# acoustic-warfare/beamforming-lk

Hardware: AMD Instinct MI355X
Metric: heatmap frames/sec (higher is better)
Workload: dtype f32

## Files before the change

### beamforming-lk_amd/csrc/awpu_handle.h

```cpp
#pragma once

#include "awpu_hip.h"
#include "awpu_hip_spectral.h"
#include "awpu_hip_track.h"

#include <hip/hip_runtime.h>

#include <algorithm>
#include <string>
#include <utility>
#include <vector>

#include "das_kernels.h"

namespace awpu::host {

void note_error(const std::string &text);

struct CtxScope {
    awpu_hip *saved;
    explicit CtxScope(awpu_hip *h);
    ~CtxScope();
};
#define AWPU_CTX(h) awpu::host::CtxScope ctx_scope_(h)
// ... 177 lines not shown
}

struct awpu_hip {
    template <class T>
    using Dev = awpu::host::DeviceBuffer<T>;
    template <class T>
    using Pinned = awpu::host::PinnedBuffer<T>;
    using Event = awpu::host::Event;
    using Stream = awpu::host::Stream;

    awpu_hip_cfg cfg{};
    Stream stream;
    Event ev_begin, ev_end;
    bool timing = true;

    std::vector<int32_t> off;
    std::vector<float> frac;
    std::vector<int32_t> index;
    std::vector<float> gain;
    bool have_table = false, have_mics = false, prepared = false;

    Dev<awpu::LutEntry> d_lut;
    struct FastLut {
        awpu::FastPlan plan;
        Dev<awpu::FastEntry> d;
        size_t entries = 0;
    };
    std::vector<FastLut> fast_luts;
    Dev<awpu::FastEntry> d_exact_pair_lut;
    size_t exact_pair_lut_entries = 0, fir_plane_lut_entries = 0;
    awpu::FastPlan exact_plan{};
    awpu::host::QuadTable quad_tables[awpu::host::kQuadLayouts];
    Dev<unsigned> d_nd_queue;
    Dev<int2> d_nd_items;
    Dev<unsigned> d_nd_starts;
    size_t nd_start_entries = 0;
    long long nd_items_key = -1;
    int n_cus = 0;
    bool exact_nd_ok = false;
    bool exact_ndh_ok = false, exact_ndhs_ok = false, fast_ndp_ok = false;
    bool identity_mics = false;
    bool exact_pairs_ok = false;
    float *sums_out = nullptr;
    Dev<uint32_t> d_fir_plane_lut;
    awpu::FastPlan fir_plane_plan{};
    bool fir_planes_ok = false;
    std::vector<float> fir;
    bool quadh_fits = false;
    bool quadhs_fits = false;
    bool quad_ok = false;
    double quad_cost = 0.0;
    double quad_differ = 3.0;
    Dev<int32_t> d_index;
    Dev<float> d_gain;
    Dev<float> d_calib;
    Dev<awpu::LutEntry> d_beam_lut;
    Dev<float> d_beam_out;
    std::vector<float> antenna;
    Dev<float> d_xyz;
    std::vector<int32_t> track_index;
    Dev<int32_t> d_track_index;
    Dev<unsigned char> d_track;
    Dev<float> d_fir;
    Dev<float> d_ring;
    Dev<uint8_t> d_display;
    Dev<awpu::ResizeTap> d_taps;
    int taps_key[4] = {0, 0, 0, 0};
// ... 63 lines not shown
};

namespace awpu::host {

enum class ExactShape : int {
    kVerify = 0,
    kDefault = 1,
    kPair = 2,
    kQuad = 3,
    kNd1 = 4,
    kNd2 = 5,
    kNdp = 6,
};
inline bool forces_exact_nd(ExactShape e) { return e == ExactShape::kNd1 || e == ExactShape::kNd2 || e == ExactShape::kNdp; }

struct EnvKnobs {
    int fpi = 0, ppw = 0, nw = 0;
    int pairs = -1;
    int debug = 0;
    int fpw = 0;
    int quads = -1;
    int pair_group = 0;
    int quad_variant = 0;
    int stationary = -1;
    int fir_planes = 1;
    int fir_share = 1;
    int wgs = 0;
    int live_graph = 1;
    int halves = -1;
    ExactShape exact_pairs = ExactShape::kDefault;
    int pair_cols = -1;
    int group_copy = 0;
    int listen_stream = 1;
    EnvKnobs();
};
const EnvKnobs &env();

struct BandSet {
    int n = 0;
    int taps[AWPU_SPECTRAL_MAX_BANDS] = {0, 0, 0, 0};
    const float *coef[AWPU_SPECTRAL_MAX_BANDS] = {nullptr, nullptr, nullptr, nullptr};
    int max_taps() const { return std::max(std::max(taps[0], taps[1]), std::max(taps[2], taps[3])); }
    int planes() const { return std::max(n, 1); }
};
inline BandSet own_band(const awpu_hip *h) {
    BandSet set;
    if (!h->band.empty()) set.n = 1, set.taps[0] = h->band_taps(), set.coef[0] = h->band.data();
    return set;
}

enum FrameLayout { kFull = 0, kCompact = 1, kRing = 2 };

int prepare(awpu_hip *h);
void free_tables(awpu_hip *h);
int launch(awpu_hip *h, const float *d_frames, int batch, float *d_power, hipStream_t s, int layout = kFull);
bool takes_packed_pairs(awpu_hip *h, int batch, awpu::FastPlan *plan);
int packed_shape(awpu_hip *h, int batch, awpu::FastPlan *plan);
size_t packed_floats_of(const awpu_hip *h, const awpu::FastPlan &plan, int batch);
int pack_for_sweep(awpu_hip *h, const awpu::FastPlan &plan, const float *d_frames, int batch, float *d_packed, hipStream_t s);
int sweep_packed(awpu_hip *h, const awpu::FastPlan &plan, const float *d_packed, size_t packed_floats, int batch, float *d_power, hipStream_t s);

void retire_live_graphs(awpu_hip *h);
int enqueue_host_process(awpu_hip *h, const float *frames, int batch, const BandSet *bands = nullptr);
int enqueue_power_to_host(awpu_hip *h, int batch, float *power, size_t pitch);
int enqueue_ingest(awpu_hip *h, const void *datagrams, int32_t stride_bytes);
int check_ready(awpu_hip *h, int batch);
// ... 52 lines not shown
```

### beamforming-lk_amd/csrc/awpu_hip.cpp

```cpp
#include "awpu_handle.h"

#include <algorithm>
#include <chrono>
#include <cmath>
#include <cstdio>
#include <cstdlib>
#include <cstring>
#include <new>
#include <string>
#include <vector>

#include "awpu_hip_band.h"
#include "band_kernels.h"
#include "band_rule.h"
#include "spectral_kernels.h"
#include "spectral_rule.h"
#include "das_kernels.h"
#include "focus_rule.h"
#include "watch_kernels.h"

using namespace awpu::host;

namespace {

// ... 3 lines not shown
}

namespace awpu::host {

void note_error(const std::string &text) {
    g_last_error = text;
    if (g_ctx) g_ctx->last_error = text;
}

CtxScope::CtxScope(awpu_hip *h) : saved(g_ctx) { g_ctx = h; }
CtxScope::~CtxScope() { g_ctx = saved; }

int hip_fail(hipError_t e, const char *what) {
    note_error(std::string(what) + ": " + hipGetErrorString(e));
    return AWPU_ERR_HIP;
}

int invalid(const char *why) {
    note_error(why);
    return AWPU_ERR_INVALID;
}

int fail(int status, const char *why) {
    note_error(why);
    return status;
}

}

awpu::host::EnvKnobs::EnvKnobs() {
    if (const char *v = std::getenv("AWPU_GROUP_FORCE_COPY")) group_copy = std::atoi(v);
    if (const char *v = std::getenv("AWPU_LIVE_GRAPH")) live_graph = std::atoi(v);
    if (const char *v = std::getenv("AWPU_SHAPE")) {
        const std::string shape(v);
        if (shape == "pair" || shape == "pair_vertical" || shape == "pair_horizontal") {
            pairs = 1, quads = 0, stationary = 0;
            if (shape != "pair") pair_cols = shape == "pair_vertical";
        } else if (shape == "quad") quads = 1;
        else if (shape == "noquad") quads = 0;
        else if (shape == "stationary") pairs = 1, quads = 0, stationary = 1;
        else if (shape == "quadh") quads = 1, pairs = 0, halves = 1;
        else if (shape == "quadh_chunked") quads = 1, pairs = 0, halves = 1, stationary = 0;
        else if (shape == "single_db") pairs = 0, quads = 0, fpi = 1, ppw = 8, nw = 32;
        else if (shape == "single_small") pairs = 0, quads = 0, fpi = 1, ppw = 2, nw = 8;
        else if (shape == "fir8_planes") fir_planes = 2;
        else if (shape == "exact_verify") exact_pairs = ExactShape::kVerify;
        else if (shape == "exact_pair") exact_pairs = ExactShape::kPair;
        else if (shape == "exact_quad") exact_pairs = ExactShape::kQuad;
        else if (shape == "exact_nd1") exact_pairs = ExactShape::kNd1;
        else if (shape == "exact_nd2") exact_pairs = ExactShape::kNd2;
        else if (shape == "exact_ndp") exact_pairs = ExactShape::kNdp;
        else std::fprintf(stderr, "libawpu_hip: AWPU_SHAPE=%s is not a shape of this build; ignored\n", v);
    }
#ifdef AWPU_TUNING_BUILD
    if (const char *v = std::getenv("AWPU_LISTEN_STREAM")) listen_stream = std::atoi(v);
    if (const char *v = std::getenv("AWPU_FAST_QUADS")) quads = std::atoi(v);
    if (const char *v = std::getenv("AWPU_FAST_PAIRGROUP")) pair_group = std::atoi(v);
    if (const char *v = std::getenv("AWPU_QUAD_VARIANT")) quad_variant = std::atoi(v);
    if (const char *v = std::getenv("AWPU_FAST_HALVES")) halves = std::atoi(v);
    if (const char *v = std::getenv("AWPU_EXACT_PAIRS")) exact_pairs = (ExactShape) std::atoi(v);
    if (const char *v = std::getenv("AWPU_FAST_WGS")) wgs = std::atoi(v);
    if (const char *v = std::getenv("AWPU_FIR8_PLANES")) fir_planes = std::atoi(v);
    if (const char *v = std::getenv("AWPU_FIR8_SHARE")) fir_share = std::atoi(v);
    if (const char *v = std::getenv("AWPU_FAST_STATIONARY")) stationary = std::atoi(v);
    if (const char *v = std::getenv("AWPU_FAST_PAIRCOLS")) pair_cols = std::atoi(v);
    if (const char *v = std::getenv("AWPU_FAST_VARIANT"))
        if (std::sscanf(v, "%d,%d,%d", &fpi, &ppw, &nw) < 2) fpi = ppw = nw = 0;
// ... 1239 lines not shown
```

### beamforming-lk_amd/csrc/awpu_sweep.cpp

```cpp
#include "awpu_handle.h"

#include <algorithm>
#include <array>
#include <cstdio>
#include <cstdlib>
#include <cstring>
#include <map>
#include <vector>

#include "das_kernels.h"
#include "nd_tile_window.h"

using namespace awpu::host;

namespace {

int diag_begin(awpu_hip *h, size_t words, bool zero, hipStream_t s, unsigned long long **out) {
    if (const int rc = h->d_diag.ensure(words); rc != AWPU_OK) return rc;
    if (zero) AWPU_HIP_TRY(hipMemsetAsync(h->d_diag, 0, words * sizeof(unsigned long long), s));
    *out = h->d_diag;
    return AWPU_OK;
}

int diag_end(awpu_hip *h, int rc, size_t n_waves, int wg_waves, const char *tag, hipStream_t s) {
// ... 440 lines not shown
    }
    if (env_fpi == 1 || env_fpi == 2) *fpi = env_fpi;
    if (env_ppw == 2 || env_ppw == 4 || env_ppw == 8) *ppw = env_ppw;
    if (env_nw == 8 || env_nw == 32 || env_nw == 24) *nw = env_nw;
    if (*nw == 32) {
        *fpi = 1;
        if (*ppw < 4) *ppw = 4;
    }
    if (*nw == 24) {
        *fpi = 1;
        *ppw = 4;
    }
    if (*fpi == 2 && *ppw == 8) *ppw = 4;
    if (*fpi == 2 && batch < 2) *fpi = 1;
}

int finish_launch(awpu_hip *h, int batch, hipStream_t s, int kernel_id) {
    h->stats.kernel_variant = kernel_id;
    if (h->timing) AWPU_HIP_TRY(hipEventRecord(h->ev_end, s));
    h->stats.launches += 1;
    h->stats.frames += (uint64_t) batch;
    return AWPU_OK;
}

int cu_count(awpu_hip *h) {
    if (h->n_cus < 1 && (hipDeviceGetAttribute(&h->n_cus, hipDeviceAttributeMultiprocessorCount, h->cfg.device) != hipSuccess || h->n_cus < 1))
        h->n_cus = 256;
    return h->n_cus;
}

int arm_item_queues(awpu_hip *h, int items, unsigned **queue, int32_t *wgs, int32_t *tail) {
    if (const int rc = h->d_nd_queue.ensure(9); rc != AWPU_OK) return rc;
    *queue = h->d_nd_queue;
    *wgs = cu_count(h);
    const int per = (items + 7) / 8;
    *tail = per >= 32 ? (per + 7) / 8 : per;
    return AWPU_OK;
}

size_t pair_pack_floats(int frames, int rows, int wr, int floats) { return (size_t) ((frames + 1) / 2) * rows * wr * floats; }

template <class Args>
void fill_shared(Args &a, const awpu_hip *h, const awpu::FastPlan &plan, int batch, float *d_power) {
    a.power = d_power;
    a.usable = h->usable();
    a.usable_pad = plan.usable_pad;
    a.pixel_count = h->cfg.pixel_count;
    a.chunk = plan.chunk;
    a.batch = batch;
}

int launch_exact_pairs(awpu_hip *h, const float *d_frames, int batch, float *d_power, hipStream_t s, int hist_eff, int wstart_eff) {
    if (const int rc = build_exact_pair_lut(h); rc != AWPU_OK) return rc;
    const awpu::FastPlan &pp = h->exact_plan;
    if (const int prc = ensure_pack(h, pair_pack_floats(std::max(h->cfg.max_batch, batch), pp.usable_pad, pp.wr, 2)); prc != AWPU_OK) return prc;
    awpu::ExactPairArgs a{};
    fill_shared(a, h, pp, batch, d_power);
    a.packed = h->d_pack;
    a.lut = h->d_exact_pair_lut;
    a.sums = h->sums_out;
    a.wp = pp.wr;
    a.cols = h->pair_cols;
    a.tiles = awpu::pair_tiles(a.pixel_count, a.cols);
    a.n_pairs = (batch + 1) / 2;
    a.pair_group = awpu::xcd_pair_group((size_t) pp.usable_pad * pp.wr * 8, a.n_pairs);
    if (h->timing) AWPU_HIP_TRY(hipEventRecord(h->ev_begin, s));
    AWPU_HIP_TRY(awpu::launch_pack_pairs(d_frames, h->cfg.n_streams, hist_eff, wstart_eff, h->d_index, h->usable(), pp.usable_pad,
// ... 580 lines not shown
```

### beamforming-lk_amd/csrc/das_fast.hip

```cpp
#include "das_kernels.h"

#include <algorithm>
#include <atomic>

namespace awpu {

typedef float f2 __attribute__((ext_vector_type(2)));
typedef float f4 __attribute__((ext_vector_type(4)));
typedef float f4u __attribute__((ext_vector_type(4), aligned(4)));
typedef float f8 __attribute__((ext_vector_type(8)));

#define AWPU_AS4 __attribute__((address_space(4)))

typedef int i16 __attribute__((ext_vector_type(16)));

struct EntryGroup {
    i16 v;
    __device__ __forceinline__ float f(int k) const { return __int_as_float(v[4 * k + 0]); }
    __device__ __forceinline__ unsigned addr(int k) const { return (unsigned) v[4 * k + 1]; }
    __device__ __forceinline__ float g(int k) const { return __int_as_float(v[4 * k + 2]); }
};

template <int FPI>
struct Reads {
// ... 159 lines not shown
}

__device__ __forceinline__ float sum8(float v) {
    v += dpp_take<0xB1>(v);
    v += dpp_take<0x4E>(v);
    v += dpp_take<0x141>(v);
    return v;
}
__device__ __forceinline__ float sum16(float v) {
    v = sum8(v);
    return v + dpp_take<0x140>(v);
}
__device__ __forceinline__ float sum32(float v) {
    v = sum16(v);
    return v + dpp_take<0x142, 0xa>(v);
}
template <int LPP>
__device__ __forceinline__ float sum_lanes(float v) {
    static_assert(LPP == 8 || LPP == 16 || LPP == 32, "groups of 8, 16 or 32 lanes");
    return LPP == 8 ? sum8(v) : LPP == 16 ? sum16(v) : sum32(v);
}
template <int LPP>
__device__ __forceinline__ constexpr int sum_lane_of(int group) {
    return LPP == 32 ? 32 * group + 16 : LPP * group;
}
__device__ __forceinline__ float lane_value(float v, int lane_index) {
    return __builtin_bit_cast(float, __builtin_amdgcn_readlane(__builtin_bit_cast(int, v), lane_index));
}

constexpr int kDppWaveRol1 = 0x134;
constexpr int kDppWaveRor1 = 0x13C;
template <int CTRL>
__device__ __forceinline__ float wave_rotate1(float v) {
    const int bits = __builtin_bit_cast(int, v);
    return __builtin_bit_cast(float, __builtin_amdgcn_update_dpp(bits, bits, CTRL, 0xf, 0xf, false));
}

__device__ __forceinline__ float finish_pixel(f2 A, f2 Q, f2 C, f2 R, float tail, int lane) {
    const float q_rot = wave_rotate1<kDppWaveRol1>(Q.x);
    const float r_rot = wave_rotate1<kDppWaveRol1>(R.x);
    const float q_next = lane == 63 ? r_rot : q_rot;
    const float r_next = lane == 63 ? tail : r_rot;
    const float o0 = A.x + Q.y;
    const float o1 = A.y + q_next;
    const float o2 = C.x + R.y;
    const float o3 = C.y + r_next;
    const float o1_prev = wave_rotate1<kDppWaveRor1>(o1);
    const float o2_next = wave_rotate1<kDppWaveRol1>(o2);
    const float o0_rot = wave_rotate1<kDppWaveRol1>(o0);
    const float o3_rot = wave_rotate1<kDppWaveRor1>(o3);
    const float o0_next = lane == 63 ? o2_next : o0_rot;
    const float o3_prev = lane == 0 ? o1_prev : o3_rot;
    const float ma0 = o0 * 0.5f - 0.25f * (o1 + o1_prev);
    const float ma1 = o1 * 0.5f - 0.25f * (o0_next + o0);
    const float ma2 = o2 * 0.5f - 0.25f * (o3 + o3_prev);
    const float ma3 = o3 * 0.5f - 0.25f * (o2_next + o2);
    float sum = ma1 * ma1 + ma2 * ma2;
    if (lane != 0) sum += ma0 * ma0;
    if (lane != 63) sum += ma3 * ma3;
    return wave_sum(sum);
}

template <int NW, int PPW, int FPI, int WPS>
__global__ __launch_bounds__(NW * 64, WPS) void das_fast_kernel(FastArgs a) {
    static_assert(PPW <= 8, "the tail pass gives 8 lanes to each of at most 8 pixels");
    extern __shared__ __attribute__((aligned(16))) float lds[];
    constexpr int FS = kFastLdsBytes / FPI;
    const int lane = threadIdx.x & 63;
// ... 854 lines not shown
    }
}

__device__ __forceinline__ f2 next_and_difference(float cur, float next, float gm) {
#pragma clang fp contract(off)
    const float c = cur * gm, n = next * gm;
    return f2{n, c - n};
}

__global__ void pack_nd_kernel(const float *frames, int n_streams, int hist, int wstart, const int32_t *index, int usable,
                               const float *gain, int wq, int batch, float *packed, unsigned *queue) {
    const int pair = blockIdx.y, s = blockIdx.x, rows_out = gridDim.x;
    if (queue && pair == 0 && s == 0 && threadIdx.x < 9) queue[threadIdx.x] = 0u;
    f4 *dst = (f4 *) packed + ((size_t) pair * rows_out + s) * wq;
    if (s >= usable) {
        for (int t = threadIdx.x; t < wq; t += blockDim.x) dst[t] = f4{0.0f, 0.0f, 0.0f, 0.0f};
        return;
    }
    const int fa = min(2 * pair, batch - 1), fb = min(2 * pair + 1, batch - 1);
    const float *xa = frames + ((size_t) fa * n_streams + index[s]) * hist + wstart;
    const float *xb = frames + ((size_t) fb * n_streams + index[s]) * hist + wstart;
    const float gm = gain ? gain[s] : 1.0f;
    const int valid = min(wq, hist - wstart - 1);
    for (int t = threadIdx.x; t < wq; t += blockDim.x) {
        f4 v = f4{0.0f, 0.0f, 0.0f, 0.0f};
        if (t < valid) {
            const f2 ea = next_and_difference(xa[t], xa[t + 1], gm), eb = next_and_difference(xb[t], xb[t + 1], gm);
            v = f4{ea.x, eb.x, ea.y, eb.y};
        }
        dst[t] = v;
    }
}

__global__ void nd_items_kernel(int2 *items, int n_pairs, int tiles, int pair_group, int tiles_per_row, int nq) {
    const int item = blockIdx.x * blockDim.x + threadIdx.x;
    if (item >= n_pairs * tiles) return;
    const int full_items = (n_pairs / pair_group) * pair_group * tiles;
    const int ga = item < full_items ? pair_group : n_pairs % pair_group;
    const int rem = item < full_items ? item : item - full_items;
    const int grp = rem / (tiles * ga), in = rem - grp * tiles * ga;
    const int tile = in / ga;
    const int pair = (item < full_items ? grp * pair_group : n_pairs - ga) + (in - tile * ga);
    const int rowq = tile / tiles_per_row, colt = tile - rowq * tiles_per_row;
    items[item] = int2{pair, (nq * rowq * tiles_per_row + colt) * 16};
}

struct NdQueues {
    unsigned *q;
    int per, total, tail;
    __device__ __forceinline__ int len(int x) const { return max(0, min(per, total - x * per)); }
    __device__ __forceinline__ int head(int x) const { return len(x) - min(len(x), tail); }
    __device__ __forceinline__ int take_head(int x) const {
        if (head(x) <= 0) return -1;
        const unsigned i = atomicAdd(&q[x], 1u);
        return i < (unsigned) head(x) ? x * per + (int) i : -1;
    }
    __device__ __forceinline__ int take_common() const {
        if (tail <= 0) return -1;
        for (;;) {
            const unsigned j = atomicAdd(&q[8], 1u);
            const int run = (int) (j / (unsigned) tail), k = (int) (j - (unsigned) run * (unsigned) tail);
            if (run >= 8) return -1;
            if (k < len(run) - head(run)) return run * per + head(run) + k;
        }
    }
    __device__ __forceinline__ int take(int xcd) const {
        int item = take_head(xcd);
        if (item < 0) item = take_common();
        for (int y = 1; item < 0 && y < 8; y++) item = take_head((xcd + y) & 7);
        return item;
    }
};

template <int NQ, bool SUMS>
__global__ __launch_bounds__(1024, 4) void das_exact_nd_kernel(ExactNdArgs a) {
    extern __shared__ __attribute__((aligned(16))) float lds[];
    constexpr int NW = 16, BUF = kFastLdsBytes;
    const int wave = __builtin_amdgcn_readfirstlane(threadIdx.x >> 6);
    const unsigned lds_base = (unsigned) (unsigned long long) (const __attribute__((address_space(3))) char *) lds;
    int *mail = (int *) (lds + 2 * (BUF / 4));
    const int total = a.n_pairs * a.tiles;
    unsigned xcc;
    asm volatile("s_getreg_b32 %0, hwreg(HW_REG_XCC_ID)" : "=s"(xcc));
    const NdQueues Q{a.queue, (total + 7) >> 3, total, a.tail};
    const int xcd = (int) (xcc & 7u);
    if (threadIdx.x == 0) {
        const int first = Q.take(xcd);
        mail[0] = first;
        mail[1] = first >= 0 ? Q.take(xcd) : -1;
    }
    __syncthreads();
    int cur = __builtin_amdgcn_readfirstlane(mail[0]), nxt = __builtin_amdgcn_readfirstlane(mail[1]);
    if (cur < 0) return;
    __syncthreads();

    const int tiles_per_row = (a.cols + NW - 1) / NW;
    auto decode = [&](int item, int &pair, int &tile_quad, const unsigned *&starts) {
        const int2 d = a.items[item];
        pair = __builtin_amdgcn_readfirstlane(d.x);
        tile_quad = __builtin_amdgcn_readfirstlane(d.y);
        const int quad_row = (tile_quad >> 4) / tiles_per_row, col_tile = (tile_quad >> 4) - quad_row * tiles_per_row;
        starts = a.starts + (size_t) ((quad_row >> 1) * tiles_per_row + col_tile) * a.usable_pad;
    };
    const int groups_total = a.usable_pad >> 2;
    const size_t row_floats = (size_t) a.wq * 4;
    const int n_chunks = (a.usable_pad + a.chunk - 1) / a.chunk;
    const int first_mics = min(a.chunk, a.usable_pad), last_mics = a.usable_pad - (n_chunks - 1) * a.chunk;
    const unsigned dbf = __builtin_amdgcn_readfirstlane((unsigned) ((size_t) a.chunk * row_floats * 4));
    const int row_bytes = a.wq_tile * 16;
    const int row_pieces = (row_bytes + 1023) >> 10;
    const unsigned last_shift = (unsigned) (row_pieces * 64 - a.wq_tile);
    const int rank = wave >> 2;
    const unsigned pka = __builtin_amdgcn_readfirstlane((unsigned) (first_mics >> 2) | (unsigned) (last_mics >> 2) << 8 | (unsigned) n_chunks << 16);
    const unsigned pkb_item = (wave < a.chunk ? (unsigned) row_pieces : 0u) | (wave < last_mics ? (unsigned) row_pieces : 0u) << 8 | last_shift << 24 |
                              (unsigned) rank << 30;
    const unsigned pkb_next = wave < first_mics ? (unsigned) row_pieces << 16 : 0u;
    const int own_head = Q.head(xcd);

    int pair, tile;
    const unsigned *starts;
    decode(cur, pair, tile, starts);
#ifdef AWPU_TUNING_BUILD
    const unsigned long long rt_begin = a.debug_out ? __builtin_amdgcn_s_memrealtime() : 0ull;
    long long t_sweep = 0, t_other = 0, t_mark = __builtin_readcyclecounter();
    int n_items = 0;
#endif
    {
        if (wave < first_mics) {
            const unsigned start = __builtin_amdgcn_readfirstlane(starts[wave]);
            const float *src = a.packed + ((size_t) pair * a.usable_pad + wave) * row_floats + (start >> 2);
            const int lane = (int) (threadIdx.x & 63);
            for (int k = 0; k < row_pieces; k++) {
                const int el = k * 64 + lane;
                if (el < a.wq_tile) {
                    float *dst = lds + ((wave * row_bytes) >> 2) + k * 256;
                    __builtin_amdgcn_global_load_lds((const __attribute__((address_space(1))) void *) (src + (size_t) el * 4),
                                                     (__attribute__((address_space(3))) void *) dst, 16, 0, 0);
                }
            }
        }
    }
    asm volatile("s_waitcnt vmcnt(0)" ::: "memory");
    __syncthreads();
    unsigned step = 0;

    for (;;) {
        const int cols_pad = tiles_per_row * NW;
        const int rowq = tile / (NQ * cols_pad);
        const int col = tile - NQ * rowq * cols_pad + wave;
        const int quad0 = tile + wave;
        const QuadEntry *quad_lut = a.lut + (size_t) quad0 * groups_total * 16;
        const float *pair_base = a.packed + (size_t) pair * a.usable_pad * row_floats;
        int pair_next = pair, tile_next = tile;
        const unsigned *starts_next = starts;
        if (nxt >= 0) decode(nxt, pair_next, tile_next, starts_next);
        const float *next_base = a.packed + (size_t) pair_next * a.usable_pad * row_floats;
        unsigned ticket = 0;
        const bool asked = wave == 0 && nxt >= 0 && own_head > 0;
        const unsigned *qptr = (const unsigned *) uniform_ptr(asked ? a.queue + xcd : nullptr);

        f8 O[NQ][4];
#ifdef AWPU_TUNING_BUILD
        { const long long n = __builtin_readcyclecounter(); t_other += n - t_mark; t_mark = n; }
#endif
        {
            unsigned tid = threadIdx.x;
            asm volatile("" : "+v"(tid));
            const unsigned lane_bytes = (tid & 63) * 16;
            const int buf = (int) (step & 1);
            unsigned lane_addr = lds_base + buf * BUF + lane_bytes;
            const unsigned ddst = __builtin_amdgcn_readfirstlane(lds_base + (buf ^ 1) * BUF + wave * row_bytes);
            const int delta = __builtin_amdgcn_readfirstlane(buf ? -BUF : BUF);
            const unsigned pkb = __builtin_amdgcn_readfirstlane(pkb_item | (nxt >= 0 ? pkb_next : 0u));
            const float *row_src = pair_base + (size_t) wave * row_floats, *row_next = next_base + (size_t) wave * row_floats;
            if constexpr (NQ == 1) {
                sweep_exact_nd_item1(O[0][0], O[0][1], O[0][2], O[0][3], uniform_ptr(quad_lut), pka, lane_addr, pkb, uniform_ptr(row_src), dbf,
                                     uniform_ptr(row_next), ddst, delta, lane_bytes, uniform_ptr(starts + wave), uniform_ptr(starts_next + wave), qptr, ticket);
            } else {
                static_assert(NQ == 2, "blocks are generated for one and two quads per wave");
                const int qstride = __builtin_amdgcn_readfirstlane(tiles_per_row * NW * groups_total * 16 * (int) sizeof(QuadEntry));
                sweep_exact_nd_item2(O[0][0], O[0][1], O[0][2], O[0][3], O[1][0], O[1][1], O[1][2], O[1][3], uniform_ptr(quad_lut), qstride, pka, lane_addr,
                                     pkb, uniform_ptr(row_src), dbf, uniform_ptr(row_next), ddst, delta, lane_bytes, uniform_ptr(starts + wave),
                                     uniform_ptr(starts_next + wave), qptr, ticket);
            }
            step += n_chunks;
        }
        if (threadIdx.x == 0 && nxt >= 0) {
            int got = own_head > 0 && ticket < (unsigned) own_head ? xcd * Q.per + (int) ticket : -1;
            if (got < 0) {
                got = Q.take_common();
                for (int y = 1; got < 0 && y < 8; y++) got = Q.take_head((xcd + y) & 7);
            }
            mail[0] = got;
        }
#ifdef AWPU_TUNING_BUILD
        { const long long n = __builtin_readcyclecounter(); t_sweep += n - t_mark; t_mark = n; n_items++; }
#endif

        unsigned tid_e = threadIdx.x;
        asm volatile("" : "+v"(tid_e));
        const int lane = (int) (tid_e & 63);
        const float norm = (float) (kSamples * a.usable);
#pragma unroll
        for (int q = 0; q < NQ; q++) {
            const int row4 = NQ * rowq + q;
            auto finish = [&](const f8 &Op, int pp) {
                const int row = 4 * row4 + pp;
                const bool live = row < a.rows && col < a.cols;
                const int p = min(row, a.rows - 1) * a.cols + min(col, a.cols - 1);
                f2 o[4];
#pragma unroll
                for (int k = 0; k < 4; k++) o[k] = f2{Op[2 * k], Op[2 * k + 1]};
                if (SUMS && live) {
#pragma unroll
                    for (int k = 0; k < 4; k++) {
                        a.sums[((size_t) (2 * pair) * a.pixel_count + p) * kSamples + lane + 64 * k] = o[k].x;
                        if (2 * pair + 1 < a.batch) a.sums[((size_t) (2 * pair + 1) * a.pixel_count + p) * kSamples + lane + 64 * k] = o[k].y;
                    }
                }
                return pixel_pair_partial_exact(o, lane);
            };
            const f2 s0 = finish(O[q][0], 0), s1 = finish(O[q][1], 1), s2 = finish(O[q][2], 2), s3 = finish(O[q][3], 3);
            const float sum = wave_sum8(s0.x, s0.y, s1.x, s1.y, s2.x, s2.y, s3.x, s3.y, lane);
            const int value = kWaveSum8Value(lane >> 3), row = 4 * row4 + (value >> 1), frame = 2 * pair + (value & 1);
            if ((lane & 7) == 0 && row < a.rows && col < a.cols && frame < a.batch)
                a.power[(size_t) frame * a.pixel_count + (size_t) row * a.cols + col] = sum / norm;
        }

        if (nxt < 0) break;
        __syncthreads();
        cur = nxt;
        pair = pair_next;
        tile = tile_next;
        starts = starts_next;
        nxt = __builtin_amdgcn_readfirstlane(mail[0]);
        __syncthreads();
    }
#ifdef AWPU_TUNING_BUILD
    if (a.debug_out && threadIdx.x == 0) {
        unsigned hw_id;
        asm volatile("s_getreg_b32 %0, hwreg(HW_REG_HW_ID)" : "=s"(hw_id));
        unsigned long long *o = a.debug_out + 8 * (size_t) blockIdx.x;
        o[0] = rt_begin;
        o[1] = __builtin_amdgcn_s_memrealtime();
        o[2] = (unsigned long long) t_other;
        o[3] = (unsigned long long) t_sweep;
        o[4] = (unsigned long long) (__builtin_readcyclecounter() - t_mark);
        o[5] = ((unsigned long long) xcc << 32) | hw_id;
        o[6] = (unsigned long long) n_items;
        o[7] = 1;
    }
#endif
}

__device__ __forceinline__ void store_tile_and_signal(float *lds, bool holder, int tile_row, int wave, int lane, float value, float *power, int row0,
                                                      int col0, int rows, int cols, const DoneFlag &done) {
    __syncthreads();
    if (holder) lds[tile_row * 16 + wave] = value;
    __syncthreads();
    if (wave != 0) return;
    const int r = row0 + (lane >> 4), c = col0 + (lane & 15);
    if (r < rows && c < cols) __hip_atomic_store(&power[(size_t) r * cols + c], lds[lane], __ATOMIC_RELAXED, __HIP_MEMORY_SCOPE_SYSTEM);
    asm volatile("s_waitcnt vmcnt(0)" ::: "memory");
    if (lane == 0 && __hip_atomic_fetch_add(done.counter, 1ull, __ATOMIC_RELAXED, __HIP_MEMORY_SCOPE_AGENT) + 1ull == done.target)
        __hip_atomic_store(done.flag, done.seq, __ATOMIC_RELAXED, __HIP_MEMORY_SCOPE_SYSTEM);
}

__global__ void pack_ndh_kernel(const float *frames, int n_streams, int pitch, int wstart, const int32_t *index, int usable,
// ... 937 lines not shown
    const int n_tiles = a.cols > 0 ? ((a.pixel_count / a.cols + 3) / 4) * ((a.cols + 15) / 16) : (a.pixel_count + 63) / 64;
    if (a.cols > 0 && (unsigned) a.wp * 2u != kFirStaticPlaneBytes) return hipErrorInvalidValue;
    if ((a.wp & 3) || a.pair_group < 1 ||
        !within({(size_t) a.pixel_count * a.usable_pad + kFir8PlaneTablePrefetch, (size_t) n_pairs * a.usable * a.wp * 2}, have))
        return hipErrorInvalidValue;
    return launch_lds<das_fir8_plane_kernel<VAR>>(xcd_grid((long) n_pairs * n_tiles), dim3(1024), kTwoImages, stream, a,
                                                  (const FirPlaneEntry *) d_entries, d_coeffs, n_tiles, a.pair_group);
}

hipError_t launch_das_fir8_planes(const PairArgs &a, const void *d_entries, const float *d_coeffs, int variant, const Extents &have,
                                  hipStream_t stream) {
#ifdef AWPU_QUAD_VARIANTS
    if (variant == 1) return launch_fir8_plane_variant<1>(a, d_entries, d_coeffs, have, stream);
    if (variant == 2) return launch_fir8_plane_variant<2>(a, d_entries, d_coeffs, have, stream);
    if (variant == 3) return launch_fir8_plane_variant<3>(a, d_entries, d_coeffs, have, stream);
#endif
    (void) variant;
    return launch_fir8_plane_variant<0>(a, d_entries, d_coeffs, have, stream);
}

hipError_t launch_pack_nd(const float *d_frames, int n_streams, int hist, int wstart, const int32_t *d_index, int usable, int rows_out,
                          const float *d_gain, int wq, int batch, float *d_packed, unsigned *d_queue, hipStream_t stream) {
    hipLaunchKernelGGL(pack_nd_kernel, dim3(rows_out, (batch + 1) / 2), dim3(128), 0, stream, d_frames, n_streams, hist, wstart, d_index,
                       usable, d_gain, wq, batch, d_packed, d_queue);
    return hipGetLastError();
}

template <int NQ, bool SUMS>
static hipError_t launch_exact_nd_variant(const ExactNdArgs &a, hipStream_t stream) {
    const long total = (long) a.n_pairs * a.tiles;
    if (!a.queue_zeroed)
        if (hipError_t e = hipMemsetAsync(a.queue, 0, 9 * sizeof(unsigned), stream); e != hipSuccess) return e;
    if (a.build_items)
        hipLaunchKernelGGL(nd_items_kernel, dim3((unsigned) ((total + 255) / 256)), dim3(256), 0, stream, const_cast<int2 *>(a.items), a.n_pairs,
                           a.tiles, a.pair_group, (a.cols + 15) / 16, NQ);
    return launch_lds<das_exact_nd_kernel<NQ, SUMS>>(dim3((unsigned) std::min<long>(total, std::max(1, a.wgs))), dim3(1024),
                                                     kTwoImages + 64, stream, a);
}

hipError_t launch_das_exact_nd(const ExactNdArgs &a, const Extents &have, hipStream_t stream) {
    if ((a.nq != 1 && a.nq != 2) || !a.queue || !a.items || a.wgs < 1 || a.tail < 1) return hipErrorInvalidValue;
    if (!chunk_fits(a.chunk, a.usable_pad, (size_t) a.wq_tile * 16) || a.chunk > 16 || a.usable < 1 || a.usable > a.usable_pad || a.wq_tile < kSamples ||
        a.wq_tile > a.wq || !grid_is(a.rows, a.cols, a.pixel_count))
        return hipErrorInvalidValue;
    if (!items_agree(a.n_pairs, a.batch, a.tiles, nd_tiles(a.rows, a.cols, a.nq), a.pair_group)) return hipErrorInvalidValue;
    if (!a.starts || a.start_entries < (size_t) nd_tiles(a.rows, a.cols, 2) * a.usable_pad + 16) return hipErrorInvalidValue;
    if (!within({(size_t) nd_quad_count(a.rows, a.cols, a.nq) * (a.usable_pad / 4) * 16 + kQuadTablePrefetch,
                 (size_t) a.n_pairs * a.usable_pad * a.wq * 4}, have))
        return hipErrorInvalidValue;
    if (a.sums) return a.nq == 2 ? launch_exact_nd_variant<2, true>(a, stream) : launch_exact_nd_variant<1, true>(a, stream);
    return a.nq == 2 ? launch_exact_nd_variant<2, false>(a, stream) : launch_exact_nd_variant<1, false>(a, stream);
}

hipError_t launch_pack_ndh(const float *d_frames, int n_streams, int pitch, int wstart, const int32_t *d_index, int usable, int rows_out,
                           const float *d_gain, int wh, int batch, float *d_packed, hipStream_t stream) {
    hipLaunchKernelGGL(pack_ndh_kernel, dim3(rows_out, batch), dim3(256), 0, stream, d_frames, n_streams, pitch, wstart, d_index, usable, d_gain,
                       wh, d_packed);
    return hipGetLastError();
}

static bool ndh_shape_ok(const ExactNdhArgs &a, int tiles_of_grid, size_t image_bytes) {
    return chunk_fits(a.chunk, a.usable_pad, (size_t) a.wh * 16, image_bytes) && a.usable >= 1 && a.usable <= a.usable_pad && a.wh >= kSamples / 2 &&
           grid_is(a.rows, a.cols, a.pixel_count) && a.batch >= 1 && a.tiles == tiles_of_grid && (long) a.batch * a.tiles <= 0x7fffffffL;
}

template <int NQ, bool STATIONARY>
static hipError_t launch_exact_ndh_variant(const ExactNdhArgs &a, hipStream_t stream) {
// ... 156 lines not shown
```

### beamforming-lk_amd/csrc/das_kernels.h

```cpp
#pragma once

#include <hip/hip_runtime.h>
#include <stdint.h>

#if defined(AWPU_TIMING_BUILD) && !defined(AWPU_TUNING_BUILD)
#define AWPU_TUNING_BUILD 1
#endif
#include "sweep_plan.h"

namespace awpu {

constexpr int kDebugNoRefill = 1, kDebugNoSweep = 2, kDebugNoTail = 4, kDebugNoBarrier = 8, kDebugRegStaging = 64;
constexpr int kDebugSafeBits = 16 | 256 | 512 | 4096;
#ifdef AWPU_TIMING_BUILD
#define AWPU_DBG(a, bit) ((a).debug & (bit))
#else
#define AWPU_DBG(a, bit) 0
#endif

struct LutEntry {
    int32_t off_rel;
    float frac;
};

// ... 68 lines not shown
    float *power;
    float *sums;
    int32_t usable, usable_pad, pixel_count, wp, chunk, batch;
    int32_t cols;
    int32_t tiles, n_pairs, pair_group;
};
hipError_t launch_das_exact_pairs(const ExactPairArgs &a, const Extents &have, hipStream_t stream);
struct ExactQuadArgs {
    const float *packed;
    const struct QuadEntry *lut;
    float *power;
    float *sums;
    int32_t usable, usable_pad, pixel_count, wp, chunk, batch;
    int32_t cols, rows;
    int32_t tiles, n_pairs, pair_group;
};
hipError_t launch_das_exact_quads(const ExactQuadArgs &a, const Extents &have, hipStream_t stream);
struct ExactNdArgs {
    const float *packed;
    const struct QuadEntry *lut;
    const unsigned *starts;
    size_t start_entries;
    int32_t wq_tile;
    float *power;
    float *sums;
    int32_t usable, usable_pad, pixel_count, wq, chunk, batch;
    int32_t cols, rows;
    int32_t nq;
    int32_t tiles, n_pairs, pair_group;
    unsigned *queue;
    int32_t queue_zeroed;
    int32_t wgs;
    int32_t tail;
    const int2 *items;
    int32_t build_items;
    unsigned long long *debug_out;
};
inline int nd_tiles(int rows, int cols, int nq) { return (((rows + 3) / 4 + nq - 1) / nq) * ((cols + 15) / 16); }
inline int nd_quad_count(int rows, int cols, int nq) { return (((rows + 3) / 4 + nq - 1) / nq) * nq * ((cols + 15) / 16) * 16; }
hipError_t launch_pack_nd(const float *d_frames, int n_streams, int hist, int wstart, const int32_t *d_index, int usable, int rows_out,
                          const float *d_gain, int wq, int batch, float *d_packed, unsigned *d_queue, hipStream_t stream);
hipError_t launch_das_exact_nd(const ExactNdArgs &a, const Extents &have, hipStream_t stream);
struct DoneFlag {
    unsigned long long *counter;
    unsigned *flag;
    unsigned long long target;
    uint32_t seq;
};
struct ExactNdhArgs {
    const float *packed;
    const float *frames;
    const struct QuadEntry *lut;
    const int32_t *index;
    const float *gain;
    float *power;
    float *sums;
    int32_t n_streams, pitch, wstart;
    int32_t usable, usable_pad, pixel_count, wh, chunk, batch;
    int32_t cols, rows;
    int32_t nq;
    int32_t tiles;
    int32_t lut_cols;
    int32_t identity;
    DoneFlag done;
};
inline int ndh_tiles(int rows, int cols, int nq) { return ((rows + 3) / 4) * ((cols + 16 * nq - 1) / (16 * nq)); }
hipError_t launch_pack_ndh(const float *d_frames, int n_streams, int pitch, int wstart, const int32_t *d_index, int usable, int rows_out,
// ... 209 lines not shown
```

Baseline: 23240.

## Precompute ND item row/start indices and rematerialize kernel args to cut SGPR pressure

Work items for the exact ND kernel widen from int2 to int4 so each item carries its quad row and start-table row precomputed, removing per-item divisions in the kernel. The persistent loop reloads scalar arguments from the kernarg segment and recomputes queue state at the item boundary instead of keeping them live. This lowers scalar register pressure across the sweep, and the next item's descriptor is fetched with a scalar load. It also uses mov_dpp in place of update_dpp for the wave rotate and adds an env knob to cap the workgroup count. The cost is a larger item table and extra scalar loads per item.

New measurement: 23410, median of 6. No clear change (+0.7%).

```diff
diff --git a/beamforming-lk_amd/csrc/awpu_handle.h b/beamforming-lk_amd/csrc/awpu_handle.h
--- a/beamforming-lk_amd/csrc/awpu_handle.h
+++ b/beamforming-lk_amd/csrc/awpu_handle.h
@@ -233,7 +233,7 @@
     awpu::FastPlan exact_plan{};
     awpu::host::QuadTable quad_tables[awpu::host::kQuadLayouts];
     Dev<unsigned> d_nd_queue;
-    Dev<int2> d_nd_items;
+    Dev<int4> d_nd_items;
     Dev<unsigned> d_nd_starts;
     size_t nd_start_entries = 0;
     long long nd_items_key = -1;
@@ -363,6 +363,7 @@
     int pair_cols = -1;
     int group_copy = 0;
     int listen_stream = 1;
+    int nd_wgs = 0;
     EnvKnobs();
 };
 const EnvKnobs &env();
diff --git a/beamforming-lk_amd/csrc/awpu_hip.cpp b/beamforming-lk_amd/csrc/awpu_hip.cpp
--- a/beamforming-lk_amd/csrc/awpu_hip.cpp
+++ b/beamforming-lk_amd/csrc/awpu_hip.cpp
@@ -59,7 +59,11 @@
     if (const char *v = std::getenv("AWPU_GROUP_FORCE_COPY")) group_copy = std::atoi(v);
     if (const char *v = std::getenv("AWPU_LIVE_GRAPH")) live_graph = std::atoi(v);
     if (const char *v = std::getenv("AWPU_SHAPE")) {
-        const std::string shape(v);
+        std::string shape(v);
+        if (const size_t cut = shape.find(":wgs="); cut != std::string::npos) {
+            nd_wgs = std::atoi(shape.c_str() + cut + 5);
+            shape.resize(cut);
+        }
         if (shape == "pair" || shape == "pair_vertical" || shape == "pair_horizontal") {
             pairs = 1, quads = 0, stationary = 0;
             if (shape != "pair") pair_cols = shape == "pair_vertical";
diff --git a/beamforming-lk_amd/csrc/awpu_sweep.cpp b/beamforming-lk_amd/csrc/awpu_sweep.cpp
--- a/beamforming-lk_amd/csrc/awpu_sweep.cpp
+++ b/beamforming-lk_amd/csrc/awpu_sweep.cpp
@@ -496,7 +496,7 @@
 int arm_item_queues(awpu_hip *h, int items, unsigned **queue, int32_t *wgs, int32_t *tail) {
     if (const int rc = h->d_nd_queue.ensure(9); rc != AWPU_OK) return rc;
     *queue = h->d_nd_queue;
-    *wgs = cu_count(h);
+    *wgs = env().nd_wgs > 0 ? std::min(env().nd_wgs, cu_count(h)) : cu_count(h);
     const int per = (items + 7) / 8;
     *tail = per >= 32 ? (per + 7) / 8 : per;
     return AWPU_OK;
diff --git a/beamforming-lk_amd/csrc/das_fast.hip b/beamforming-lk_amd/csrc/das_fast.hip
--- a/beamforming-lk_amd/csrc/das_fast.hip
+++ b/beamforming-lk_amd/csrc/das_fast.hip
@@ -215,8 +215,7 @@
 constexpr int kDppWaveRor1 = 0x13C;
 template <int CTRL>
 __device__ __forceinline__ float wave_rotate1(float v) {
-    const int bits = __builtin_bit_cast(int, v);
-    return __builtin_bit_cast(float, __builtin_amdgcn_update_dpp(bits, bits, CTRL, 0xf, 0xf, false));
+    return __builtin_bit_cast(float, __builtin_amdgcn_mov_dpp(__builtin_bit_cast(int, v), CTRL, 0xf, 0xf, false));
 }
 
 __device__ __forceinline__ float finish_pixel(f2 A, f2 Q, f2 C, f2 R, float tail, int lane) {
@@ -1137,7 +1136,7 @@
     }
 }
 
-__global__ void nd_items_kernel(int2 *items, int n_pairs, int tiles, int pair_group, int tiles_per_row, int nq) {
+__global__ void nd_items_kernel(int4 *items, int n_pairs, int tiles, int pair_group, int tiles_per_row, int nq) {
     const int item = blockIdx.x * blockDim.x + threadIdx.x;
     if (item >= n_pairs * tiles) return;
     const int full_items = (n_pairs / pair_group) * pair_group * tiles;
@@ -1147,7 +1146,7 @@
     const int tile = in / ga;
     const int pair = (item < full_items ? grp * pair_group : n_pairs - ga) + (in - tile * ga);
     const int rowq = tile / tiles_per_row, colt = tile - rowq * tiles_per_row;
-    items[item] = int2{pair, (nq * rowq * tiles_per_row + colt) * 16};
+    items[item] = int4{pair, (nq * rowq * tiles_per_row + colt) * 16, 4 * nq * rowq, ((nq * rowq) >> 1) * tiles_per_row + colt};
 }
 
 struct NdQueues {
@@ -1199,15 +1198,12 @@
     if (cur < 0) return;
     __syncthreads();
 
-    const int tiles_per_row = (a.cols + NW - 1) / NW;
-    auto decode = [&](int item, int &pair, int &tile_quad, const unsigned *&starts) {
-        const int2 d = a.items[item];
+    auto place = [&](const int4 d, int &pair, int &tile_quad, int &row0, int &start_row) {
         pair = __builtin_amdgcn_readfirstlane(d.x);
         tile_quad = __builtin_amdgcn_readfirstlane(d.y);
-        const int quad_row = (tile_quad >> 4) / tiles_per_row, col_tile = (tile_quad >> 4) - quad_row * tiles_per_row;
-        starts = a.starts + (size_t) ((quad_row >> 1) * tiles_per_row + col_tile) * a.usable_pad;
+        row0 = __builtin_amdgcn_readfirstlane(d.z);
+        start_row = __builtin_amdgcn_readfirstlane(d.w);
     };
-    const int groups_total = a.usable_pad >> 2;
     const size_t row_floats = (size_t) a.wq * 4;
     const int n_chunks = (a.usable_pad + a.chunk - 1) / a.chunk;
     const int first_mics = min(a.chunk, a.usable_pad), last_mics = a.usable_pad - (n_chunks - 1) * a.chunk;
@@ -1217,14 +1213,15 @@
     const unsigned last_shift = (unsigned) (row_pieces * 64 - a.wq_tile);
     const int rank = wave >> 2;
     const unsigned pka = __builtin_amdgcn_readfirstlane((unsigned) (first_mics >> 2) | (unsigned) (last_mics >> 2) << 8 | (unsigned) n_chunks << 16);
-    const unsigned pkb_item = (wave < a.chunk ? (unsigned) row_pieces : 0u) | (wave < last_mics ? (unsigned) row_pieces : 0u) << 8 | last_shift << 24 |
-                              (unsigned) rank << 30;
-    const unsigned pkb_next = wave < first_mics ? (unsigned) row_pieces << 16 : 0u;
-    const int own_head = Q.head(xcd);
-
-    int pair, tile;
-    const unsigned *starts;
-    decode(cur, pair, tile, starts);
+    const unsigned pkb_item = __builtin_amdgcn_readfirstlane((wave < a.chunk ? (unsigned) row_pieces : 0u) |
+                                                             (wave < last_mics ? (unsigned) row_pieces : 0u) << 8 | last_shift << 24 | (unsigned) rank << 30);
+    const unsigned pkb_next = __builtin_amdgcn_readfirstlane(wave < first_mics ? (unsigned) row_pieces << 16 : 0u);
+    const unsigned *q_own = (const unsigned *) uniform_ptr(wave == 0 && Q.head(xcd) > 0 ? a.queue + xcd : nullptr);
+
+    int pair, tile, row0, start_row;
+    place(a.items[cur], pair, tile, row0, start_row);
+    int pair_next = pair, tile_next = tile, row0_next = row0, start_row_next = start_row;
+    if (nxt >= 0) place(a.items[nxt], pair_next, tile_next, row0_next, start_row_next);
 #ifdef AWPU_TUNING_BUILD
     const unsigned long long rt_begin = a.debug_out ? __builtin_amdgcn_s_memrealtime() : 0ull;
     long long t_sweep = 0, t_other = 0, t_mark = __builtin_readcyclecounter();
@@ -1232,7 +1229,7 @@
 #endif
     {
         if (wave < first_mics) {
-            const unsigned start = __builtin_amdgcn_readfirstlane(starts[wave]);
+            const unsigned start = __builtin_amdgcn_readfirstlane(a.starts[(size_t) start_row * a.usable_pad + wave]);
             const float *src = a.packed + ((size_t) pair * a.usable_pad + wave) * row_floats + (start >> 2);
             const int lane = (int) (threadIdx.x & 63);
             for (int k = 0; k < row_pieces; k++) {
@@ -1250,19 +1247,19 @@
     unsigned step = 0;
 
     for (;;) {
-        const int cols_pad = tiles_per_row * NW;
-        const int rowq = tile / (NQ * cols_pad);
-        const int col = tile - NQ * rowq * cols_pad + wave;
+        const auto *kp = (const __attribute__((address_space(4))) ExactNdArgs *) __builtin_amdgcn_kernarg_segment_ptr();
+        asm volatile("" : "+s"(kp));
+        const int usable_pad = kp->usable_pad, groups_total = usable_pad >> 2;
+        const size_t row_floats = (size_t) kp->wq * 4;
+        const float *const packed = kp->packed;
+        const unsigned *const start_table = kp->starts;
         const int quad0 = tile + wave;
-        const QuadEntry *quad_lut = a.lut + (size_t) quad0 * groups_total * 16;
-        const float *pair_base = a.packed + (size_t) pair * a.usable_pad * row_floats;
-        int pair_next = pair, tile_next = tile;
-        const unsigned *starts_next = starts;
-        if (nxt >= 0) decode(nxt, pair_next, tile_next, starts_next);
-        const float *next_base = a.packed + (size_t) pair_next * a.usable_pad * row_floats;
+        const QuadEntry *quad_lut = kp->lut + (size_t) quad0 * groups_total * 16;
+        const float *pair_base = packed + (size_t) pair * usable_pad * row_floats;
+        const unsigned *starts = start_table + (size_t) start_row * usable_pad, *starts_next = start_table + (size_t) start_row_next * usable_pad;
+        const float *next_base = packed + (size_t) pair_next * usable_pad * row_floats;
         unsigned ticket = 0;
-        const bool asked = wave == 0 && nxt >= 0 && own_head > 0;
-        const unsigned *qptr = (const unsigned *) uniform_ptr(asked ? a.queue + xcd : nullptr);
+        const unsigned *qptr = nxt >= 0 ? q_own : nullptr;
 
         f8 O[NQ][4];
 #ifdef AWPU_TUNING_BUILD
@@ -1276,51 +1273,64 @@
             unsigned lane_addr = lds_base + buf * BUF + lane_bytes;
             const unsigned ddst = __builtin_amdgcn_readfirstlane(lds_base + (buf ^ 1) * BUF + wave * row_bytes);
             const int delta = __builtin_amdgcn_readfirstlane(buf ? -BUF : BUF);
-            const unsigned pkb = __builtin_amdgcn_readfirstlane(pkb_item | (nxt >= 0 ? pkb_next : 0u));
+            const unsigned pkb = pkb_item | (nxt >= 0 ? pkb_next : 0u);
             const float *row_src = pair_base + (size_t) wave * row_floats, *row_next = next_base + (size_t) wave * row_floats;
             if constexpr (NQ == 1) {
                 sweep_exact_nd_item1(O[0][0], O[0][1], O[0][2], O[0][3], uniform_ptr(quad_lut), pka, lane_addr, pkb, uniform_ptr(row_src), dbf,
                                      uniform_ptr(row_next), ddst, delta, lane_bytes, uniform_ptr(starts + wave), uniform_ptr(starts_next + wave), qptr, ticket);
             } else {
                 static_assert(NQ == 2, "blocks are generated for one and two quads per wave");
-                const int qstride = __builtin_amdgcn_readfirstlane(tiles_per_row * NW * groups_total * 16 * (int) sizeof(QuadEntry));
+                const int qstride = ((kp->cols + NW - 1) / NW) * NW * groups_total * 16 * (int) sizeof(QuadEntry);
                 sweep_exact_nd_item2(O[0][0], O[0][1], O[0][2], O[0][3], O[1][0], O[1][1], O[1][2], O[1][3], uniform_ptr(quad_lut), qstride, pka, lane_addr,
                                      pkb, uniform_ptr(row_src), dbf, uniform_ptr(row_next), ddst, delta, lane_bytes, uniform_ptr(starts + wave),
                                      uniform_ptr(starts_next + wave), qptr, ticket);
             }
             step += n_chunks;
         }
-        if (threadIdx.x == 0 && nxt >= 0) {
-            int got = own_head > 0 && ticket < (unsigned) own_head ? xcd * Q.per + (int) ticket : -1;
-            if (got < 0) {
-                got = Q.take_common();
-                for (int y = 1; got < 0 && y < 8; y++) got = Q.take_head((xcd + y) & 7);
-            }
-            mail[0] = got;
+        const auto *ka = (const __attribute__((address_space(4))) ExactNdArgs *) __builtin_amdgcn_kernarg_segment_ptr();
+        asm volatile("" : "+s"(ka));
+        unsigned tid_e = threadIdx.x;
+        int nxt_e = nxt;
+        asm volatile("" : "+v"(tid_e), "+s"(nxt_e));
+        if (__builtin_amdgcn_readfirstlane(tid_e >> 6) == 0 && nxt_e >= 0) {
+            unsigned xcc_e;
+            asm volatile("s_getreg_b32 %0, hwreg(HW_REG_XCC_ID)" : "=s"(xcc_e));
+            const int xcd_e = (int) (xcc_e & 7u), total_e = ka->n_pairs * ka->tiles;
+            const NdQueues Qe{ka->queue, (total_e + 7) >> 3, total_e, ka->tail};
+            const int own_head_e = Qe.head(xcd_e);
+            if (tid_e == 0) {
+                int got = own_head_e > 0 && ticket < (unsigned) own_head_e ? xcd_e * Qe.per + (int) ticket : -1;
+                if (got < 0) {
+                    got = Qe.take_common();
+                    for (int y = 1; got < 0 && y < 8; y++) got = Qe.take_head((xcd_e + y) & 7);
+                }
+                mail[0] = got;
+            }
         }
 #ifdef AWPU_TUNING_BUILD
         { const long long n = __builtin_readcyclecounter(); t_sweep += n - t_mark; t_mark = n; n_items++; }
 #endif
 
-        unsigned tid_e = threadIdx.x;
-        asm volatile("" : "+v"(tid_e));
-        const int lane = (int) (tid_e & 63);
-        const float norm = (float) (kSamples * a.usable);
+        const int lane = (int) (tid_e & 63), wave_e = __builtin_amdgcn_readfirstlane(tid_e >> 6);
+        const int rows = ka->rows, cols = ka->cols, batch = ka->batch, pixel_count = ka->pixel_count;
+        float *const power = ka->power;
+        const float norm = (float) (kSamples * ka->usable);
+        const int col = tile - (row0 >> 2) * (((cols + NW - 1) / NW) * NW) + wave_e;
 #pragma unroll
         for (int q = 0; q < NQ; q++) {
-            const int row4 = NQ * rowq + q;
+            const int row4 = (row0 >> 2) + q;
             auto finish = [&](const f8 &Op, int pp) {
                 const int row = 4 * row4 + pp;
-                const bool live = row < a.rows && col < a.cols;
-                const int p = min(row, a.rows - 1) * a.cols + min(col, a.cols - 1);
+                const bool live = row < rows && col < cols;
+                const int p = min(row, rows - 1) * cols + min(col, cols - 1);
                 f2 o[4];
 #pragma unroll
                 for (int k = 0; k < 4; k++) o[k] = f2{Op[2 * k], Op[2 * k + 1]};
                 if (SUMS && live) {
 #pragma unroll
                     for (int k = 0; k < 4; k++) {
-                        a.sums[((size_t) (2 * pair) * a.pixel_count + p) * kSamples + lane + 64 * k] = o[k].x;
-                        if (2 * pair + 1 < a.batch) a.sums[((size_t) (2 * pair + 1) * a.pixel_count + p) * kSamples + lane + 64 * k] = o[k].y;
+                        a.sums[((size_t) (2 * pair) * pixel_count + p) * kSamples + lane + 64 * k] = o[k].x;
+                        if (2 * pair + 1 < batch) a.sums[((size_t) (2 * pair + 1) * pixel_count + p) * kSamples + lane + 64 * k] = o[k].y;
                     }
                 }
                 return pixel_pair_partial_exact(o, lane);
@@ -1328,17 +1338,23 @@
             const f2 s0 = finish(O[q][0], 0), s1 = finish(O[q][1], 1), s2 = finish(O[q][2], 2), s3 = finish(O[q][3], 3);
             const float sum = wave_sum8(s0.x, s0.y, s1.x, s1.y, s2.x, s2.y, s3.x, s3.y, lane);
             const int value = kWaveSum8Value(lane >> 3), row = 4 * row4 + (value >> 1), frame = 2 * pair + (value & 1);
-            if ((lane & 7) == 0 && row < a.rows && col < a.cols && frame < a.batch)
-                a.power[(size_t) frame * a.pixel_count + (size_t) row * a.cols + col] = sum / norm;
-        }
-
-        if (nxt < 0) break;
+            if ((lane & 7) == 0 && row < rows && col < cols && frame < batch)
+                power[(size_t) frame * pixel_count + (size_t) row * cols + col] = sum / norm;
+        }
+
+        if (nxt_e < 0) break;
         __syncthreads();
         cur = nxt;
         pair = pair_next;
         tile = tile_next;
-        starts = starts_next;
+        row0 = row0_next;
+        start_row = start_row_next;
         nxt = __builtin_amdgcn_readfirstlane(mail[0]);
+        if (nxt >= 0) {
+            typedef int i4 __attribute__((ext_vector_type(4)));
+            const i4 r = ((const __attribute__((address_space(4))) i4 *) (unsigned long long) ka->items)[nxt];
+            pair_next = r.x, tile_next = r.y, row0_next = r.z, start_row_next = r.w;
+        }
         __syncthreads();
     }
 #ifdef AWPU_TUNING_BUILD
@@ -2342,7 +2358,7 @@
     if (!a.queue_zeroed)
         if (hipError_t e = hipMemsetAsync(a.queue, 0, 9 * sizeof(unsigned), stream); e != hipSuccess) return e;
     if (a.build_items)
-        hipLaunchKernelGGL(nd_items_kernel, dim3((unsigned) ((total + 255) / 256)), dim3(256), 0, stream, const_cast<int2 *>(a.items), a.n_pairs,
+        hipLaunchKernelGGL(nd_items_kernel, dim3((unsigned) ((total + 255) / 256)), dim3(256), 0, stream, const_cast<int4 *>(a.items), a.n_pairs,
                            a.tiles, a.pair_group, (a.cols + 15) / 16, NQ);
     return launch_lds<das_exact_nd_kernel<NQ, SUMS>>(dim3((unsigned) std::min<long>(total, std::max(1, a.wgs))), dim3(1024),
                                                      kTwoImages + 64, stream, a);
diff --git a/beamforming-lk_amd/csrc/das_kernels.h b/beamforming-lk_amd/csrc/das_kernels.h
--- a/beamforming-lk_amd/csrc/das_kernels.h
+++ b/beamforming-lk_amd/csrc/das_kernels.h
@@ -124,7 +124,7 @@
     int32_t queue_zeroed;
     int32_t wgs;
     int32_t tail;
-    const int2 *items;
+    const int4 *items;
     int32_t build_items;
     unsigned long long *debug_out;
 };
```
